# schreibfaul1/ESP32-Opus-Player

Measured on AMD Instinct MI355X. Metric: decoded 48 kHz stereo frames/sec/GPU (x real-time); HBM GB/s vs roofline, higher is better.
Workload: dtype int32 fixed-point (int16/int32 with 64-bit products); 1 GPU; celt_fb_stereo_64k; streams_per_gpu=65536

## Files before the change

### esp32-opus-player_amd/csrc/og_celt_packed.hpp

```cpp
#pragma once
#include <stddef.h>
#include "og_celt_bands.hpp"

namespace og {

#if defined(OG_RECON_TIGHT) && !defined(OG_HOST_EMUL)
constexpr bool PM_PACKED = true;
#else
constexpr bool PM_PACKED = false;
#endif

#ifdef OG_HOST_EMUL
OG_DEV u32 pk_perm(u32 hi, u32 lo, u32 sel) {
    const u64 v = (u64)hi << 32 | lo;
    u32 r = 0;
    for (int b = 0; b < 4; b++) r |= (u32)((v >> (8 * ((sel >> (8 * b)) & 7u))) & 0xffu) << (8 * b);
    return r;
}
OG_DEV i32 pk_dot2(u32 a, u32 b, i32 acc) {
    return (i32)((u32)acc + (u32)((i32)(i16)a * (i32)(i16)b) + (u32)(((i32)a >> 16) * ((i32)b >> 16)));
}
OG_DEV i32 pk_dot2_fits(u32 a, u32 b, i32 acc) { return pk_dot2(a, b, acc); }
OG_DEV u32 pk_add16(u32 a, u32 b) { return ((a + b) & 0xffffu) | ((a & 0xffff0000u) + (b & 0xffff0000u)); }
OG_DEV u32 pk_sub16(u32 a, u32 b) { return ((a - b) & 0xffffu) | ((a & 0xffff0000u) - (b & 0xffff0000u)); }
#else
typedef unsigned short og_u16x2 __attribute__((ext_vector_type(2)));
OG_DEV u32 pk_perm(u32 hi, u32 lo, u32 sel) { return __builtin_amdgcn_perm(hi, lo, sel); }
OG_DEV i32 pk_dot2(u32 a, u32 b, i32 acc) { return rs_dot2(a, b, acc); }
OG_DEV i32 pk_dot2_fits(u32 a, u32 b, i32 acc) {
    return __builtin_amdgcn_sdot2(__builtin_bit_cast(og_i16x2, a), __builtin_bit_cast(og_i16x2, b), acc, true);
}
OG_DEV u32 pk_add16(u32 a, u32 b) { return __builtin_bit_cast(u32, __builtin_bit_cast(og_u16x2, a) + __builtin_bit_cast(og_u16x2, b)); }
OG_DEV u32 pk_sub16(u32 a, u32 b) { return __builtin_bit_cast(u32, __builtin_bit_cast(og_u16x2, a) - __builtin_bit_cast(og_u16x2, b)); }
#endif
OG_DEV u32 pk_lolo(u32 a, u32 b) { return pk_perm(b, a, 0x05040100u); }
OG_DEV u32 pk_hihi(u32 a, u32 b) { return pk_perm(b, a, 0x07060302u); }
OG_DEV u32 pk_pair(i32 lo, i32 hi) { return ((u32)lo & 0xffffu) | (u32)hi << 16; }
OG_DEV u32 pk_q15(i32 lo, i32 hi) { return (((u32)lo >> 15) & 0xffffu) | (((u32)hi << 1) & 0xffff0000u); }
OG_DEV u32 pk_shr(i32 lo, i32 hi, int s) { return pk_pair(lo >> s, hi >> s); }

struct W4 { u32 w[4]; };
#ifdef OG_HOST_EMUL
template <typename T>
OG_DEV T pk_ld(const i16 *p) {
    T v;
    memcpy(&v, p, sizeof(T));
    return v;
}
OG_DEV W4 ldw4(const i16 *p) { return pk_ld<W4>(p); }
OG_DEV void stw4(i16 *p, const W4 &r) { memcpy(p, &r, sizeof(r)); }
#else
typedef i32 og_v4i __attribute__((ext_vector_type(4)));
template <typename T>
OG_DEV T pk_ld(const i16 *p) { return *reinterpret_cast<const T *>(p); }
OG_DEV W4 ldw4(const i16 *p) {
    const og_v4i v = *reinterpret_cast<const og_v4i *>(p);
    return W4{{(u32)v.x, (u32)v.y, (u32)v.z, (u32)v.w}};
}
OG_DEV void stw4(i16 *p, const W4 &r) { *reinterpret_cast<og_v4i *>(p) = og_v4i{(i32)r.w[0], (i32)r.w[1], (i32)r.w[2], (i32)r.w[3]}; }
#endif

#ifdef OG_HOST_EMUL
struct W2 { u32 w[2]; };
#else
struct alignas(8) W2 { u32 w[2]; };
#endif

constexpr u32 HAAR_SUM = 23170u | 23170u << 16, HAAR_DIF = 23170u | (u32)(u16)(-23170) << 16;
OG_DEV void pk_haar_words(u32 &x, u32 &y) {
    const u32 p = pk_lolo(x, y), q = pk_hihi(x, y);
    x = pk_q15(pk_dot2_fits(p, HAAR_SUM, 16384), pk_dot2_fits(q, HAAR_SUM, 16384));
    y = pk_q15(pk_dot2_fits(p, HAAR_DIF, 16384), pk_dot2_fits(q, HAAR_DIF, 16384));
}
OG_DEV void pk_haar8_1(W4 &r) {
    i32 s[4], d[4];
#pragma unroll
    for (int m = 0; m < 4; m++) {
        s[m] = pk_dot2_fits(r.w[m], HAAR_SUM, 16384);
        d[m] = pk_dot2_fits(r.w[m], HAAR_DIF, 16384);
    }
#pragma unroll
    for (int m = 0; m < 4; m++) r.w[m] = pk_q15(s[m], d[m]);
}
OG_DEV void pk_haar8_2(W4 &r) { pk_haar_words(r.w[0], r.w[1]); pk_haar_words(r.w[2], r.w[3]); }
OG_DEV void pk_haar8_4(W4 &r) { pk_haar_words(r.w[0], r.w[2]); pk_haar_words(r.w[1], r.w[3]); }
OG_DEV void pk_haar16(W4 &a, W4 &b) {
#pragma unroll
    for (int m = 0; m < 4; m++) pk_haar_words(a.w[m], b.w[m]);
}

static_assert(V_X % 8 == 0 && 960 % 8 == 0, "a channel's spectrum starts 16-byte aligned, its bands at multiples of 8 coefficients");
OG_DEV W4 pk_gather(const i16 *x, int N, int gj, int ls, bool had) {
    W4 r;
    if (ls == 2) {
        const int n0 = N >> 2;
        const i16 *p = x + 2 * gj;
        const u32 r0 = pk_ld<u32>(p + (had ? 3 : 0) * n0), r1 = pk_ld<u32>(p + (had ? 0 : 1) * n0);
        const u32 r2 = pk_ld<u32>(p + 2 * n0), r3 = pk_ld<u32>(p + (had ? 1 : 3) * n0);
        r.w[0] = pk_lolo(r0, r1);
        r.w[1] = pk_lolo(r2, r3);
        r.w[2] = pk_hihi(r0, r1);
        r.w[3] = pk_hihi(r2, r3);
    } else if (ls == 3) {
        const int n0 = N >> 3;
        const i16 *p = x + gj;
        const u32 rows = had ? 0x25163407u : 0x76543210u;
#pragma unroll
        for (int m = 0; m < 4; m++)
            r.w[m] = (u32)pk_ld<u16>(p + (int)((rows >> (8 * m)) & 15u) * n0) | (u32)pk_ld<u16>(p + (int)((rows >> (8 * m + 4)) & 15u) * n0) << 16;
    } else if (ls == 1) {
        const int n0 = N >> 1;
        const i16 *p = x + 4 * gj;
        const W2 a = pk_ld<W2>(p + (had ? n0 : 0)), b = pk_ld<W2>(p + (had ? 0 : n0));
        r.w[0] = pk_lolo(a.w[0], b.w[0]);
        r.w[1] = pk_hihi(a.w[0], b.w[0]);
        r.w[2] = pk_lolo(a.w[1], b.w[1]);
        r.w[3] = pk_hihi(a.w[1], b.w[1]);
    } else {
        const int stride = 1 << ls, n0 = N >> ls;
        i32 v[8];
#pragma unroll
        for (int k = 0; k < 8; k++) {
            const int inter = 8 * gj + k, j = inter >> ls, i = inter & (stride - 1);
            v[k] = x[(had ? ordery(stride, i) : i) * n0 + j];
        }
#pragma unroll
        for (int m = 0; m < 4; m++) r.w[m] = pk_pair(v[2 * m], v[2 * m + 1]);
    }
    return r;
}

OG_DEV void pk_merge_sums(const W4 &a, const W4 &b, i32 &xp, i32 &side) {
#pragma unroll
    for (int m = 0; m < 4; m++) {
        xp = pk_dot2(b.w[m], a.w[m], xp);
        side = pk_dot2(b.w[m], b.w[m], side);
    }
}
OG_DEV void pk_merge_apply(W4 &a, W4 &b, i32 mid, i32 lgain, i32 rgain, int kl, int kr, bool inv) {
    const u32 m_lo = (u32)mid & 0xffffu, m_hi = (u32)mid << 16;
    const u32 l_lo = (u32)lgain & 0xffffu, l_hi = (u32)lgain << 16, r_lo = (u32)rgain & 0xffffu, r_hi = (u32)rgain << 16;
    const i32 rl = (1 << (kl + 1)) >> 1, rr = (1 << (kr + 1)) >> 1;
#pragma unroll
    for (int m = 0; m < 4; m++) {
        const u32 l = pk_q15(pk_dot2_fits(a.w[m], m_lo, 16384), pk_dot2_fits(a.w[m], m_hi, 16384));
        const u32 d = pk_sub16(l, b.w[m]), s = pk_add16(l, b.w[m]);
        a.w[m] = pk_shr(pk_dot2_fits(d, l_lo, rl), pk_dot2_fits(d, l_hi, rl), kl + 1);
        const u32 y = pk_shr(pk_dot2_fits(s, r_lo, rr), pk_dot2_fits(s, r_hi, rr), kr + 1);
        b.w[m] = inv ? pk_sub16(0u, y) : y;
    }
}
OG_DEV W4 pk_neg(const W4 &a) { return W4{{pk_sub16(0u, a.w[0]), pk_sub16(0u, a.w[1]), pk_sub16(0u, a.w[2]), pk_sub16(0u, a.w[3])}}; }

static_assert(RING % 8 == 0 && 120 % 8 == 0 && OVERLAP / 2 % 4 == 0, "ring pieces of 4 samples: whole, and never across the wrap");
static_assert(offsetof(CeltState, ring) % 16 == 0 && offsetof(CeltState, tail) % 16 == 0 && sizeof(CeltState) % 16 == 0 &&
              sizeof(((CeltState *)nullptr)->tail[0]) % 16 == 0, "the ring and the tails are 16-byte aligned");
static_assert(V_SYN % 8 == 0, "the synthesis buffer is 16-byte aligned in the working set");
struct P4 { i32 v[4]; };
OG_DEV P4 pk_ld4(const i32 *p) {
#ifdef OG_HOST_EMUL
    P4 r;
    memcpy(&r, p, sizeof(r));
    return r;
#else
    const og_v4i v = *reinterpret_cast<const og_v4i *>(p);
    return P4{{v.x, v.y, v.z, v.w}};
#endif
}
OG_DEV void pk_st4(i32 *p, const P4 &r) {
#ifdef OG_HOST_EMUL
    memcpy(p, &r, sizeof(r));
#else
    *reinterpret_cast<og_v4i *>(p) = og_v4i{r.v[0], r.v[1], r.v[2], r.v[3]};
#endif
}
OG_DEV void pk_ring_tail_store(i32 *ring, i32 *tail, const i32 *sy, int pos, int n) {
    OG_FOR_LANES(p, n / 4) pk_st4(&ring[(pos + 4 * p) & RING_MASK], pk_ld4(&sy[4 * p]));
    OG_FOR_LANES(p, OVERLAP / 2 / 4) pk_st4(&tail[4 * p], pk_ld4(&sy[n + 4 * p]));
}

}
```

### esp32-opus-player_amd/csrc/og_celt_recon_pm.hpp

```cpp
#pragma once

namespace og {

struct PmLds {
    u32 jdesc[2 * NBANDS];
    u32 jaux[2 * NBANDS];
    u32 bw0[NBANDS], bw1[NBANDS], bw2[NBANDS];
    i32 scale[NBANDS];
    u32 mpar[NBANDS][2];
    u16 jcm[2 * NBANDS];
    u8 binband[100], binoff[100];
};
#ifdef OG_RECON_TIGHT
constexpr int V_PART = V_IY;
static_assert(sizeof(PmLds) <= sizeof(i16) * (V_IY - V_NORM) && 800 <= sizeof(i16) * (V_WIN - V_IY), "the phase-major tables");
#else
constexpr int V_PART = V_NORM + 600;
static_assert(sizeof(PmLds) <= sizeof(i16) * 600 && 600 + 400 <= 1248, "the phase-major tables overlay the folding-history rows");
#endif
OG_DEV PmLds &PM() { return *reinterpret_cast<PmLds *>(&S.v[V_NORM]); }
typedef i32 PmPart[2];
OG_DEV PmPart *pm_part() { return reinterpret_cast<PmPart *>(&S.v[V_PART]); }

enum {
    JD_VALID = 1, JD_FILL = 2,
    JD_PERM_SHIFT = 2 , JD_HAD = 1 << 5,
    JD_STEP_SHIFT = 8
};

struct V8 { i32 v[8]; };
OG_DEV V8 ld8(int pos) {
    V8 r;
#ifdef OG_HOST_EMUL
    for (int k = 0; k < 8; k++) r.v[k] = S.v[pos + k];
#else
    const og_v4i p = *reinterpret_cast<const og_v4i *>(&S.v[pos]);
    r.v[0] = (i32)(i16)p.x; r.v[1] = p.x >> 16; r.v[2] = (i32)(i16)p.y; r.v[3] = p.y >> 16;
    r.v[4] = (i32)(i16)p.z; r.v[5] = p.z >> 16; r.v[6] = (i32)(i16)p.w; r.v[7] = p.w >> 16;
#endif
    return r;
}
OG_DEV void st8(int pos, const V8 &r) {
#ifdef OG_HOST_EMUL
    for (int k = 0; k < 8; k++) S.v[pos + k] = (i16)r.v[k];
#else
    og_v4i p;
    p.x = (i32)(((u32)r.v[0] & 0xffffu) | (u32)r.v[1] << 16); p.y = (i32)(((u32)r.v[2] & 0xffffu) | (u32)r.v[3] << 16);
    p.z = (i32)(((u32)r.v[4] & 0xffffu) | (u32)r.v[5] << 16); p.w = (i32)(((u32)r.v[6] & 0xffffu) | (u32)r.v[7] << 16);
    *reinterpret_cast<og_v4i *>(&S.v[pos]) = p;
#endif
}
OG_DEV void haar_pair(i32 &a, i32 &b) {
    const i32 t1 = mul16(23170, a), t2 = mul16(23170, b);
    a = tr16(pshr32(t1 + t2, 15));
    b = tr16(pshr32(t1 - t2, 15));
}
template <int S_>
OG_DEV void haar8(V8 &r) {
#pragma unroll
    for (int i = 0; i < 8; i++)
        if (!(i & S_)) haar_pair(r.v[i], r.v[i + S_]);
}

template <bool PACKED> struct PmHold { typedef V8 type; };
template <> struct PmHold<true> { typedef W4 type; };

struct PmGrp { int band, job, x, gj, N; u32 jd; };
constexpr int PM_GROUPS = 100;
OG_DEV PmGrp pm_group(int g) {
    const PmLds &P = PM();
    PmGrp r;
    const int ch = g >= PM_GROUPS, bin = g - PM_GROUPS * ch;
    r.band = P.binband[bin];
    r.gj = P.binoff[bin];
    r.job = 2 * r.band + ch;
    r.jd = P.jdesc[r.job];
    r.x = V_X + 960 * ch + 8 * (bin - r.gj);
    r.N = (int)(P.bw1[r.band] >> 22) & 255;
    return r;
}

OG_DEV u32 pm_setup_jobs(const ParseRec *rec, int C, int B, u32 &fill_lo, u32 &fill_hi, int &dual_end, int start = 0, bool bw_staged = false) {
    PmLds &P = PM();
    OG_LSYNC();
    OG_FOR_LANES(bin, PM_GROUPS) {
        P.binband[bin] = rom_bin2band[bin];
        P.binoff[bin] = rom_binoff[bin];
    }
    OG_FOR_LANES(i, 2 * NBANDS) {
        P.jdesc[i] = 0;
        P.jcm[i] = 0;
    }
    OG_LSYNC();
    u32 tfm = 0, flo = 0, fhi = 0, de = 0;
    const int logBf = ilog2(B);
    OG_FOR_LANES(l, 2 * NBANDS) {
        const int band = l >> 1, jb = l & 1, coded = band >= start;
#ifdef OG_RECON_TIGHT
        const int bw = !coded ? 0 : bw_staged ? (int)S.band_w_row()[band] : (int)rec->band_w[band];
#else
        const int bw = coded ? (int)rec->band_w[band] : 0;
#endif
        const u32 *wp = rec->words + bw;
        const u32 w0 = coded ? wp[0] : 0u, w1 = coded ? wp[1] : 0u, w2 = coded ? wp[2] : 0u, w3 = coded ? wp[3] : 0u, jw0 = coded ? wp[4] : 0u;
        const int N = (int)(w1 >> 22) & 255;
        const int stereo = (w0 & BW_STEREO) != 0, dual = (w0 & BW_DUAL) != 0, mid_first = (w0 & BW_MID_FIRST) != 0;
        const int njobs = !coded ? 0 : (stereo || dual) ? 2 : 1;
        if (jb == 0) {
            P.bw0[band] = w0;
            P.bw1[band] = w1;
            P.bw2[band] = w2;
            P.scale[band] = (i32)(i16)(w3 & 0xffff);
            if (w0 & BW_DUAL_END) de |= 1u << band;
        }
        const int exists = jb < njobs;
        const int ch = dual ? jb : stereo ? (((jb == 0) == mid_first) ? 0 : 1) : 0;
        const int jpos = bw + 4 + (jb ? 1 + 2 * (int)(jw0 & 31) : 0);
        u32 jw = jw0;
        if (jb && exists) jw = rec->words[OG_MIN(jpos, REC_WORDS_CAP - 1)];
        const int n_fill = (int)(jw & 31), n_pvq = (int)(jw >> JW_NPVQ_SHIFT) & 31;
        P.jaux[l] = (u32)jpos | (u32)ch << 16 | (u32)exists << 17 | (u32)(exists && n_fill > 0) << 18 | (u32)(n_pvq > 0) << 19;
        if (exists) {
            int tf_change = (int)((w0 >> BW_TF_SHIFT) & 7) - 4;
            int recombine = tf_change > 0 ? tf_change : 0, time_divide = 0;
            int logB = logBf - recombine, N_B = (N >> logBf) << recombine;
            while ((N_B & 1) == 0 && tf_change < 0) {
                logB++;
                N_B >>= 1;
                time_divide++;
                tf_change++;
            }
            const int logB0 = logB;
            u32 jd = JD_VALID;
            if (logB0 > 0) jd |= (u32)(logB0 + recombine) << JD_PERM_SHIFT | (B == 1 ? JD_HAD : 0);
            int step = 0;
            for (int k = 0; k < time_divide; k++, step++) jd |= (u32)(logB0 - 1 - k + 1) << (JD_STEP_SHIFT + 4 * step);
            for (int k = 0; k < recombine; k++, step++) jd |= (u32)(k + 1) << (JD_STEP_SHIFT + 4 * step);
            if (n_fill > 0) {
                jd |= JD_FILL;
                if (l < 32) flo |= 1u << l; else fhi |= 1u << (l - 32);
            } else {
                if (logB0 > 0) tfm |= 1u;
                for (int k = 0; k < 3; k++) {
                    const int c = (int)(jd >> (JD_STEP_SHIFT + 4 * k)) & 15;
                    if (c) tfm |= 1u << (1 + 4 * k + (c - 1));
                }
                u32 cm = n_pvq ? S.job_mask_row()[l] : 0u;
                for (int k = 0; k < time_divide; k++) {
                    logB--;
                    cm |= cm >> (1 << logB);
                }
                for (int k = 0; k < recombine; k++) {
                    const u32 c4 = cm & 0xF;
                    cm = ((c4 & 1) * 0x03) | ((c4 >> 1 & 1) * 0x0C) | ((c4 >> 2 & 1) * 0x30) | ((c4 >> 3 & 1) * 0xC0);
                }
                logB += recombine;
                P.jcm[2 * band + ch] = (u16)(cm & ((1u << (1 << logB)) - 1));
            }
            P.jdesc[2 * band + ch] = jd;
        }
    }
    tfm = wave_or(tfm);
    fill_lo = wave_or(flo);
    fill_hi = wave_or(fhi);
    de = wave_or(de);
    dual_end = de ? ilog2((i32)de) : NBANDS + 1;
    OG_LSYNC();
    return tfm;
}

template <bool PACKED = PM_PACKED>
OG_DEV void pm_tf_undo(u32 tfm) {
    constexpr int NG = (2 * PM_GROUPS + OG_NLANES - 1) / OG_NLANES;
    typedef typename PmHold<PACKED>::type Hold;
    if (tfm & 1u) {
        Hold hold[NG];
        u8 mark[NG];
#pragma unroll
        for (int it = 0; it < NG; it++) {
            const int g = OG_LANE + it * OG_NLANES;
            mark[it] = 0;
            if (g < 2 * PM_GROUPS) {
                const PmGrp q = pm_group(g);
                const int ls = (int)(q.jd >> JD_PERM_SHIFT) & 7;
                if ((q.jd & JD_VALID) && !(q.jd & JD_FILL) && ls) {
                    const int stride = 1 << ls, n0 = q.N >> ls, had = (q.jd & JD_HAD) != 0;
                    if constexpr (PACKED)
                        hold[it] = pk_gather(&S.v[q.x], q.N, q.gj, ls, had);
                    else {
#pragma unroll
                        for (int k = 0; k < 8; k++) {
                            const int inter = 8 * q.gj + k, j = inter >> ls, i = inter & (stride - 1);
                            hold[it].v[k] = S.v[q.x + (had ? ordery(stride, i) : i) * n0 + j];
                        }
                    }
                    mark[it] = 1;
                }
            }
        }
        OG_LSYNC();
#pragma unroll
        for (int it = 0; it < NG; it++) {
            const int g = OG_LANE + it * OG_NLANES;
            if (mark[it]) {
                const PmGrp q = pm_group(g);
                if constexpr (PACKED) stw4(&S.v[q.x + 8 * q.gj], hold[it]);
                else st8(q.x + 8 * q.gj, hold[it]);
            }
        }
        OG_LSYNC();
    }
    if (tfm & (1u << (1 + 3))) {
#pragma unroll
        for (int it = 0; it < NG; it++) {
            const int g = OG_LANE + it * OG_NLANES;
            if (g < 2 * PM_GROUPS) {
                const PmGrp q = pm_group(g);
                if ((q.jd & JD_VALID) && !(q.jd & JD_FILL) && ((q.jd >> JD_STEP_SHIFT) & 15) == 4 && !(q.gj & 1)) {
                    if constexpr (PACKED) {
                        W4 a = ldw4(&S.v[q.x + 8 * q.gj]), b = ldw4(&S.v[q.x + 8 * q.gj + 8]);
                        pk_haar16(a, b);
                        stw4(&S.v[q.x + 8 * q.gj], a);
                        stw4(&S.v[q.x + 8 * q.gj + 8], b);
                    } else {
                        V8 a = ld8(q.x + 8 * q.gj), b = ld8(q.x + 8 * q.gj + 8);
#pragma unroll
                        for (int k = 0; k < 8; k++) haar_pair(a.v[k], b.v[k]);
                        st8(q.x + 8 * q.gj, a);
                        st8(q.x + 8 * q.gj + 8, b);
                    }
                }
            }
        }
        OG_LSYNC();
    }
    if (tfm & 0x0eeeu) {
#pragma unroll
        for (int it = 0; it < NG; it++) {
            const int g = OG_LANE + it * OG_NLANES;
            if (g < 2 * PM_GROUPS) {
                const PmGrp q = pm_group(g);
                const u32 steps = (q.jd & JD_VALID) && !(q.jd & JD_FILL) ? (q.jd >> JD_STEP_SHIFT) & 0xfffu : 0u;
                if (steps & 0x777u) {
                    if constexpr (PACKED) {
                        W4 r = ldw4(&S.v[q.x + 8 * q.gj]);
                        for (int k = 0; k < 3; k++) {
                            const int c = (int)(steps >> (4 * k)) & 15;
                            if (c == 1) pk_haar8_1(r);
                            else if (c == 2) pk_haar8_2(r);
                            else if (c == 3) pk_haar8_4(r);
                        }
                        stw4(&S.v[q.x + 8 * q.gj], r);
                    } else {
                        V8 r = ld8(q.x + 8 * q.gj);
                        for (int k = 0; k < 3; k++) {
                            const int c = (int)(steps >> (4 * k)) & 15;
                            if (c == 1) haar8<1>(r);
                            else if (c == 2) haar8<2>(r);
                            else if (c == 3) haar8<4>(r);
                        }
                        st8(q.x + 8 * q.gj, r);
                    }
                }
            }
        }
        OG_LSYNC();
    }
}

OG_DEV void pm_make_lowband(int dst, int p0, int n, int i, int use_y, int dual_end, int norm_offset = 0, int dup_n1 = 0, int dup_back = 0) {
    const PmLds &P = PM();
    OG_LSYNC();
    OG_FOR_LANES(j, n) {
        int r = p0 + j;
        const bool copied = dup_back && r >= dup_n1;
        if (copied) r -= dup_back;
        const int p = norm_offset + r, sb = P.binband[p >> 3];
        const i32 sc = P.scale[sb];
        i32 v;
        if (i >= dual_end && sb < dual_end && !copied)
            v = ((i32)(i16)mul16_q15(sc, S.v[V_X + p]) + (i32)(i16)mul16_q15(sc, S.v[V_X + 960 + p])) >> 1;
        else
            v = mul16_q15(sc, S.v[V_X + (use_y ? 960 : 0) + p]);
        S.v[dst + j] = (i16)v;
    }
    OG_LSYNC();
}

OG_DEV u32 pm_band_cm(int b, int c) {
    const PmLds &P = PM();
    const u32 w0 = (u32)OG_UNI(P.bw0[b]);
    if (w0 & BW_STEREO) return (u32)OG_UNI(P.jcm[2 * b]) | (u32)OG_UNI(P.jcm[2 * b + 1]);
    return (u32)OG_UNI(P.jcm[2 * b + ((w0 & BW_DUAL) ? c : 0)]);
}

OG_DEV void pm_fill_jobs(const u32 *words, const LcgTab &lcg, u32 fill_lo, u32 fill_hi, int C, int B, int dual_end, u32 &seed,
                         int start = 0) {
    const int norm_offset = 8 * rom_eband[start];
    const int dup_n1 = 8 * (rom_eband[start + 1] - rom_eband[start]), dup_n2 = 8 * (rom_eband[start + 2] - rom_eband[start + 1]);
    PmLds &P = PM();
    RecCur cur;
    cur.words = words;
    cur.w = 0;
    cur.base = -64;
    cur.leaf = 0;
    for (int l = 0; l < 2 * NBANDS; l++) {
        if (!((l < 32 ? fill_lo >> l : fill_hi >> (l - 32)) & 1u)) continue;
        OG_MARK(5);
        OG_STAT(20, 1);
        const int i = l >> 1, jb = l & 1;
        const u32 aux = (u32)OG_UNI(P.jaux[l]), w0 = (u32)OG_UNI(P.bw0[i]), w1 = (u32)OG_UNI(P.bw1[i]);
        const int ch = (int)(aux >> 16) & 1;
        const int eb0 = (int)(w1 >> 11) & 2047, N = (int)(w1 >> 22) & 255;
        const int tf_change = (int)((w0 >> BW_TF_SHIFT) & 7) - 4;
        const int stereo = (w0 & BW_STEREO) != 0, dual = (w0 & BW_DUAL) != 0;
        u32 x_cm, y_cm;
        if (w0 & BW_HAS_LOW) {
            const int fold_end = (int)(w0 >> BW_FOLD1_SHIFT) & 31;
            int fold_i = (int)(w0 >> BW_FOLD0_SHIFT) & 31;
            x_cm = y_cm = 0;
            do {
                x_cm |= pm_band_cm(fold_i, 0);
                y_cm |= pm_band_cm(fold_i, C - 1);
            } while (++fold_i < fold_end);
        } else
            x_cm = y_cm = (1u << B) - 1;
        i32 jfill;
        int want_low;
        if (dual) {
            jfill = (i32)(jb ? y_cm : x_cm);
            want_low = 1;
        } else {
            i32 fill0 = (i32)(x_cm | y_cm);
            if (stereo) {
                if (w0 & BW_THETA0) fill0 &= (1 << B) - 1;
                if (w0 & BW_THETA1) fill0 &= ((1 << B) - 1) << B;
            }
            jfill = ch ? fill0 >> B : fill0;
            want_low = !ch;
        }
        if (jfill == 0 && !(OG_UNI(P.jaux[l]) >> 19 & 1)) {
            OG_STAT(24, 1);
            continue;
        }
        cur.w = (int)(aux & 0xffff);
        OG_STAT(27, 1);
        const u32 jw = rec_word(cur);
        int low = -1;
        if ((w0 & BW_HAS_LOW) && want_low && (jw & JW_NEED_LOW)) {
            const int dup = (i == start + 1 && dup_n2 > dup_n1) ? dup_n2 - dup_n1 : 0;
            pm_make_lowband(V_IY, (int)(w1 & 2047), N, i, dual && ch, dual_end, norm_offset, dup_n1, dup);
            low = V_IY;
        }
        const u32 cm = recon_band_mono(cur, jw, lcg, tf_change, seed, V_X + 960 * ch + eb0, N, B, low, -1, 0, -1, jfill, l);
        if (OG_LANE == 0) P.jcm[2 * i + ch] = (u16)cm;
        OG_LSYNC();
    }
}

template <bool PACKED = PM_PACKED>
OG_DEV void pm_stereo_merge(int C) {
    PmLds &P = PM();
    if (C != 2) return;
    OG_LSYNC();
    const int eb_lo = rom_eband[OG_MIN(OG_LANE, NBANDS - 1)], eb_hi = rom_eband[OG_MIN(OG_LANE, NBANDS - 1) + 1];
    OG_FOR_LANES(g, PM_GROUPS) {
        const int band = P.binband[g];
        if (P.bw0[band] & BW_STEREO) {
            OG_STAT(29, 1);
            i32 xp = 0, side = 0;
            if constexpr (PACKED)
                pk_merge_sums(ldw4(&S.v[V_X + 8 * g]), ldw4(&S.v[V_X + 960 + 8 * g]), xp, side);
            else {
                const V8 a = ld8(V_X + 8 * g), b = ld8(V_X + 960 + 8 * g);
#pragma unroll
                for (int k = 0; k < 8; k++) {
                    xp += mul16(b.v[k], a.v[k]);
                    side += mul16(b.v[k], b.v[k]);
                }
            }
            pm_part()[g][0] = xp;
            pm_part()[g][1] = side;
        }
    }
    OG_LSYNC();
    OG_FOR_LANES(band, NBANDS) {
        const u32 w0 = P.bw0[band];
        if (w0 & BW_STEREO) {
            const int g0 = OG_NLANES > 1 ? eb_lo : rom_eband[band], g1 = OG_NLANES > 1 ? eb_hi : rom_eband[band + 1];
            i32 xp = 0, side = 0;
            for (int g = g0; g < g1; g++) {
                xp += pm_part()[g][0];
                side += pm_part()[g][1];
            }
            const i32 mid = (i32)(i16)(P.bw2[band] & 0xffff);
            xp = mul16x32_q15(mid, xp);
            const i32 mid2 = tr16(mid >> 1);
            const i32 El = mul16(mid2, mid2) + side - 2 * xp, Er = mul16(mid2, mid2) + side + 2 * xp;
            i32 mode = 1, lgain = 0, rgain = 0;
            int kl = 0, kr = 0;
            if (Er < 161061 || El < 161061)
                mode = 2;
            else {
                kl = ilog2(El) >> 1;
                kr = ilog2(Er) >> 1;
                lgain = rsqrt_norm(vshr32(El, (kl - 7) << 1));
                rgain = rsqrt_norm(vshr32(Er, (kr - 7) << 1));
                if (kl < 7) kl = 7;
                if (kr < 7) kr = 7;
            }
            if (w0 & BW_INV) mode |= 4;
            P.mpar[band][0] = (u32)(mode | kl << 8 | kr << 16);
            P.mpar[band][1] = ((u32)lgain & 0xffffu) | (u32)rgain << 16;
        } else
            P.mpar[band][0] = 0u;
    }
    OG_LSYNC();
    OG_FOR_LANES(g, PM_GROUPS) {
        const int band = P.binband[g];
        const i32 m0 = (i32)P.mpar[band][0];
        if (m0 & 3) {
            const u32 m1 = P.mpar[band][1];
            const i32 lgain = (i32)(i16)(m1 & 0xffff), rgain = (i32)m1 >> 16, mid = (i32)(i16)(P.bw2[band] & 0xffff);
            const int kl = (m0 >> 8) & 255, kr = (m0 >> 16) & 255;
            OG_STAT(37, 1);
            OG_STAT(38, (m0 & 2) != 0);
            if constexpr (PACKED) {
                W4 a = ldw4(&S.v[V_X + 8 * g]), b;
                if (m0 & 2)
                    b = (m0 & 4) ? pk_neg(a) : a;
                else {
                    b = ldw4(&S.v[V_X + 960 + 8 * g]);
                    pk_merge_apply(a, b, mid, lgain, rgain, kl, kr, (m0 & 4) != 0);
                    stw4(&S.v[V_X + 8 * g], a);
                }
                stw4(&S.v[V_X + 960 + 8 * g], b);
            } else {
                V8 a = ld8(V_X + 8 * g), b = ld8(V_X + 960 + 8 * g);
#pragma unroll
                for (int k = 0; k < 8; k++) {
                    i32 xo, yo;
                    if (m0 & 2) {
                        xo = a.v[k];
                        yo = a.v[k];
                    } else {
                        const i32 l = tr16(mul16_p15(mid, a.v[k])), r = b.v[k];
                        xo = tr16(pshr32(mul16(lgain, sub16(l, r)), kl + 1));
                        yo = tr16(pshr32(mul16(rgain, add16(l, r)), kr + 1));
                    }
                    a.v[k] = xo;
                    b.v[k] = (m0 & 4) ? tr16(-yo) : yo;
                }
                if (!(m0 & 2)) st8(V_X + 8 * g, a);
                st8(V_X + 960 + 8 * g, b);
            }
        }
    }
    OG_LSYNC();
}

OG_DEV void recon_all_bands_pm(const ParseRec *rec, LcgTab &lcg, int C, int shortBlocks, u32 &seed_io, int start = 0, bool bw_staged = false) {
    const int B = shortBlocks ? 8 : 1;
    u32 fill_lo, fill_hi, seed = seed_io;
    int dual_end;
    OG_MARK(3);
    const u32 tfm = pm_setup_jobs(rec, C, B, fill_lo, fill_hi, dual_end, start, bw_staged);
    if (fill_lo | fill_hi) lcg.hold();
#if defined(OG_HOST_EMUL) && defined(OG_STATS)
    {
        int n_fill_jobs = 0, w_prev = -1;
        bool close_pair = false;
        for (int l = 0; l < 2 * NBANDS; l++)
            if ((l < 32 ? fill_lo >> l : fill_hi >> (l - 32)) & 1u) {
                const int w = (int)(PM().jaux[l] & 0xffff);
                close_pair |= w_prev >= 0 && w - w_prev < 64;
                w_prev = w;
                n_fill_jobs++;
            }
        OG_STAT(33, n_fill_jobs == 0);
        OG_STAT(34, n_fill_jobs == 1);
        OG_STAT(35, n_fill_jobs >= 4);
        OG_STAT(36, close_pair);
    }
    {
        OG_STAT(25, (tfm & (1u << 4)) != 0);
        OG_STAT(28, (tfm & 0x0eeeu) != 0);
        for (int l = 0; l < 2 * NBANDS; l++) {
            const u32 jd = PM().jdesc[l];
            const int groups = (int)((PM().bw1[l >> 1] >> 22) & 255) / 8;
            if (!(jd & JD_VALID) || !(jd & ~(u32)(JD_VALID | JD_FILL))) continue;
            if (jd & JD_FILL) {
                OG_STAT(60, groups);
                continue;
            }
            const u32 steps = (jd >> JD_STEP_SHIFT) & 0xfffu;
            const int ls = (int)(jd >> JD_PERM_SHIFT) & 7, had = (jd & JD_HAD) != 0;
            OG_STAT(ls == 2 && had && steps == 0x012u ? 39
                    : ls == 3 && had && steps == 0x123u ? 43
                    : ls == 0 && steps == 0x321u ? 47
                    : ls == 3 && !had && steps == 0x001u ? 48
                    : ls == 3 && !had && steps == 0u ? 49
                    : ls == 4 && !had && steps == 0x004u ? 54
                    : 55, groups);
        }
    }
#endif
    OG_STAT(0, 1);
    OG_STAT(19, shortBlocks != 0);
    OG_STAT(21, tfm != 0);
    OG_STAT(22, (tfm & 1u) != 0);
    OG_STAT(23, (fill_lo | fill_hi) != 0);
    OG_MARK(8);
    if (tfm) pm_tf_undo(tfm);
    if (fill_lo | fill_hi) pm_fill_jobs(rec->words, lcg, fill_lo, fill_hi, C, B, dual_end, seed, start);
    OG_MARK(10);
    pm_stereo_merge(C);
    OG_MARK(4);
    OG_FOR_LANES(t, NBANDS * C) {
        const PmLds &P = PM();
        const int b = t / C, c = t - b * C;
        const u32 w0 = P.bw0[b];
        const u32 cm = (w0 & BW_STEREO) ? (u32)P.jcm[2 * b] | (u32)P.jcm[2 * b + 1] : (u32)P.jcm[2 * b + ((w0 & BW_DUAL) ? c : 0)];
        S.cmask_row()[t] = (u8)cm;
    }
    OG_LSYNC();
    seed_io = seed;
}

#ifdef OG_RECON_TIGHT
static_assert(sizeof(i32) * 2 * PM_GROUPS <= offsetof(PmLds, binband), "the groups' sums end before the bin tables");
static_assert(48 + 2 * 2 * NBANDS <= 200 && (V_TMP + 48) % 2 == 0, "r and the entries' words fit the scratch row");
OG_DEV void anti_collapse_pm(const LcgTab &lcg, int LM, int C, int size, int start, int end, u32 seed) {
    const PmLds &P = PM();
    const i16 *const rrow = anti_collapse_r(LM, C, start, end);
    u32 *const ent = reinterpret_cast<u32 *>(&S.v[V_TMP + 48]);
    i32 *const part = reinterpret_cast<i32 *>(&S.v[V_NORM]);
    const int NE = C * NBANDS;
    OG_STAT(32, 1);
    u32 run = 0;
    (void)run;
    OG_FOR_LANES(e, OG_NLANES > 1 ? OG_NLANES : NE) {
        const int i = C == 2 ? e >> 1 : e;
        int draws = 0;
        if (e < NE && i >= start && i < end) {
            const int cnt = __builtin_popcount(~(u32)S.cmask_row()[e] & 0xffu);
            draws = cnt * (rom_eband[i + 1] - rom_eband[i]);
            OG_STAT(30, cnt);
            OG_STAT(31, cnt != 0);
        }
#ifdef OG_HOST_EMUL
        const u32 before = run;
        run += (u32)draws;
#else
        const u32 before = (u32)(wave_scan_add(draws) - draws);
#endif
        if (e < NE) ent[e] = lcg_skip(seed, before);
    }
    OG_LSYNC();
    OG_FOR_LANES(t, C * PM_GROUPS) {
        const int c = t >= PM_GROUPS, g = t - PM_GROUPS * c;
        const int i = P.binband[g], j = P.binoff[g], e = i * C + c;
        const u32 clr = (i >= start && i < end) ? ~(u32)S.cmask_row()[e] & 0xffu : 0u;
        if (clr) {
            const int N0 = rom_eband[i + 1] - rom_eband[i];
            const i32 r = rrow[c * NBANDS + i];
            const u32 base = ent[e];
            V8 x = ld8(V_X + c * size + 8 * g);
            int at = j;
            i32 ss = 0;
#pragma unroll
            for (int k = 0; k < 8; k++) {
                const u32 s = lcg.at(base, at);
                if ((clr >> k) & 1u) {
                    x.v[k] = (i16)((s & 0x8000) ? r : -r);
                    at += N0;
                }
                ss += mul16(x.v[k], x.v[k]);
            }
            st8(V_X + c * size + 8 * g, x);
            part[t] = ss;
        }
    }
    OG_LSYNC();
    OG_FOR_LANES(e, NE) {
        const int i = C == 2 ? e >> 1 : e, c = e - i * C;
        u32 w = 0;
        if (i >= start && i < end && (~(u32)S.cmask_row()[e] & 0xffu)) {
            const int g0 = rom_eband[i], g1 = rom_eband[i + 1];
            i32 E = 1;
            for (int g = g0; g < g1; g++) E += part[c * PM_GROUPS + g];
            const int k = ilog2(E) >> 1;
            const i32 t = vshr32(E, 2 * (k - 7));
            const i32 gn = tr16(mul16_p15(rsqrt_norm(t), 32767));
            w = ((u32)gn & 0xffffu) | (u32)((k + 1) & 63) << 16 | 1u << 31;
        }
        ent[e] = w;
    }
    OG_LSYNC();
    OG_FOR_LANES(t, C * PM_GROUPS) {
        const int c = t >= PM_GROUPS, g = t - PM_GROUPS * c;
        const u32 w = ent[P.binband[g] * C + c];
        if (w) {
            const i32 gn = (i32)(i16)(w & 0xffff);
            const int sh = (int)(w >> 16) & 63;
            V8 x = ld8(V_X + c * size + 8 * g);
#pragma unroll
            for (int k = 0; k < 8; k++) x.v[k] = (i16)pshr32(mul16(gn, x.v[k]), sh);
            st8(V_X + c * size + 8 * g, x);
        }
    }
    OG_LSYNC();
}
#endif

}
```

Before: 52.50 million frames/s.

## Route fill-job band TF transforms through packed group-wise haar/permute path

In packed mode, fill jobs no longer call recon_band_mono. They plan the TF recombine/time-divide themselves, apply the forward haar and permute to the lowband in 8-coefficient groups using packed dot2 ops, and decode the leaves. They then undo the TF transform per job with group-wise gather, haar and scatter, and rebuild the collapse mask from the plan. This replaces the generic scalar per-coefficient TF loops with vectorized packed LDS accesses, at the cost of extra barriers and a new scatter path. The change also refactors pm_tf_undo onto shared helpers and adds a host-only census instrument.

```diff
diff --git a/esp32-opus-player_amd/csrc/og_celt_packed.hpp b/esp32-opus-player_amd/csrc/og_celt_packed.hpp
--- a/esp32-opus-player_amd/csrc/og_celt_packed.hpp
+++ b/esp32-opus-player_amd/csrc/og_celt_packed.hpp
@@ -130,6 +130,45 @@
     return r;
 }
 
+#ifdef OG_HOST_EMUL
+template <typename T>
+OG_DEV void pk_st(i16 *p, const T &v) { memcpy(p, &v, sizeof(T)); }
+#else
+template <typename T>
+OG_DEV void pk_st(i16 *p, const T &v) { *reinterpret_cast<T *>(p) = v; }
+#endif
+OG_DEV void pk_scatter(i16 *x, int N, int gj, int ls, bool had, const W4 &r) {
+    if (ls == 2) {
+        const int n0 = N >> 2;
+        i16 *p = x + 2 * gj;
+        pk_st<u32>(p + (had ? 3 : 0) * n0, pk_lolo(r.w[0], r.w[2]));
+        pk_st<u32>(p + (had ? 0 : 1) * n0, pk_hihi(r.w[0], r.w[2]));
+        pk_st<u32>(p + 2 * n0, pk_lolo(r.w[1], r.w[3]));
+        pk_st<u32>(p + (had ? 1 : 3) * n0, pk_hihi(r.w[1], r.w[3]));
+    } else if (ls == 3) {
+        const int n0 = N >> 3;
+        i16 *p = x + gj;
+        const u32 rows = had ? 0x25163407u : 0x76543210u;
+#pragma unroll
+        for (int m = 0; m < 4; m++) {
+            pk_st<u16>(p + (int)((rows >> (8 * m)) & 15u) * n0, (u16)r.w[m]);
+            pk_st<u16>(p + (int)((rows >> (8 * m + 4)) & 15u) * n0, (u16)(r.w[m] >> 16));
+        }
+    } else if (ls == 1) {
+        const int n0 = N >> 1;
+        i16 *p = x + 4 * gj;
+        pk_st<W2>(p + (had ? n0 : 0), W2{{pk_lolo(r.w[0], r.w[1]), pk_lolo(r.w[2], r.w[3])}});
+        pk_st<W2>(p + (had ? 0 : n0), W2{{pk_hihi(r.w[0], r.w[1]), pk_hihi(r.w[2], r.w[3])}});
+    } else {
+        const int stride = 1 << ls, n0 = N >> ls;
+#pragma unroll
+        for (int k = 0; k < 8; k++) {
+            const int inter = 8 * gj + k, j = inter >> ls, i = inter & (stride - 1);
+            x[(had ? ordery(stride, i) : i) * n0 + j] = (i16)(u16)(r.w[k >> 1] >> (16 * (k & 1)));
+        }
+    }
+}
+
 OG_DEV void pk_merge_sums(const W4 &a, const W4 &b, i32 &xp, i32 &side) {
 #pragma unroll
     for (int m = 0; m < 4; m++) {
diff --git a/esp32-opus-player_amd/csrc/og_celt_recon_pm.hpp b/esp32-opus-player_amd/csrc/og_celt_recon_pm.hpp
--- a/esp32-opus-player_amd/csrc/og_celt_recon_pm.hpp
+++ b/esp32-opus-player_amd/csrc/og_celt_recon_pm.hpp
@@ -1,4 +1,8 @@
 #pragma once
+
+#if defined(OG_HOST_EMUL) && defined(OG_STATS) && defined(OG_FILL_CENSUS)
+extern long long og_fill_census[32];
+#endif
 
 namespace og {
 
@@ -62,8 +66,60 @@
         if (!(i & S_)) haar_pair(r.v[i], r.v[i + S_]);
 }
 
-template <bool PACKED> struct PmHold { typedef V8 type; };
-template <> struct PmHold<true> { typedef W4 type; };
+template <bool PACKED> struct PmHold {
+    typedef V8 type;
+    static OG_MEMBER V8 ld(int pos) { return ld8(pos); }
+    static OG_MEMBER V8 gather(int x, int N, int gj, int ls, bool had) {
+        const int stride = 1 << ls, n0 = N >> ls;
+        V8 r;
+#pragma unroll
+        for (int k = 0; k < 8; k++) {
+            const int inter = 8 * gj + k, j = inter >> ls, i = inter & (stride - 1);
+            r.v[k] = S.v[x + (had ? ordery(stride, i) : i) * n0 + j];
+        }
+        return r;
+    }
+};
+template <> struct PmHold<true> {
+    typedef W4 type;
+    static OG_MEMBER W4 ld(int pos) { return ldw4(&S.v[pos]); }
+    static OG_MEMBER W4 gather(int x, int N, int gj, int ls, bool had) { return pk_gather(&S.v[x], N, gj, ls, had); }
+};
+OG_DEV void pm_grp_st(int pos, const V8 &r) { st8(pos, r); }
+OG_DEV void pm_grp_st(int pos, const W4 &r) { stw4(&S.v[pos], r); }
+OG_DEV void pm_grp_scatter(int x, int N, int gj, int ls, bool had, const V8 &r) {
+    const int stride = 1 << ls, n0 = N >> ls;
+#pragma unroll
+    for (int k = 0; k < 8; k++) {
+        const int inter = 8 * gj + k, j = inter >> ls, i = inter & (stride - 1);
+        S.v[x + (had ? ordery(stride, i) : i) * n0 + j] = (i16)r.v[k];
+    }
+}
+OG_DEV void pm_grp_scatter(int x, int N, int gj, int ls, bool had, const W4 &r) { pk_scatter(&S.v[x], N, gj, ls, had, r); }
+OG_DEV V8 pm_grp_steps(V8 r, u32 steps) {
+    for (int k = 0; k < 3; k++) {
+        const int c = (int)(steps >> (4 * k)) & 15;
+        if (c == 1) haar8<1>(r);
+        else if (c == 2) haar8<2>(r);
+        else if (c == 3) haar8<4>(r);
+    }
+    return r;
+}
+OG_DEV W4 pm_grp_steps(W4 r, u32 steps) {
+    for (int k = 0; k < 3; k++) {
+        const int c = (int)(steps >> (4 * k)) & 15;
+        if (c == 1) pk_haar8_1(r);
+        else if (c == 2) pk_haar8_2(r);
+        else if (c == 3) pk_haar8_4(r);
+    }
+    return r;
+}
+OG_DEV u32 pm_steps_reversed(u32 steps) { return (steps & 0x0f0u) | (steps >> 8 & 15u) | (steps & 15u) << 8; }
+OG_DEV void pm_grp_pair(V8 &a, V8 &b) {
+#pragma unroll
+    for (int k = 0; k < 8; k++) haar_pair(a.v[k], b.v[k]);
+}
+OG_DEV void pm_grp_pair(W4 &a, W4 &b) { pk_haar16(a, b); }
 
 struct PmGrp { int band, job, x, gj, N; u32 jd; };
 constexpr int PM_GROUPS = 100;
@@ -172,7 +228,8 @@
 template <bool PACKED = PM_PACKED>
 OG_DEV void pm_tf_undo(u32 tfm) {
     constexpr int NG = (2 * PM_GROUPS + OG_NLANES - 1) / OG_NLANES;
-    typedef typename PmHold<PACKED>::type Hold;
+    typedef PmHold<PACKED> G;
+    typedef typename G::type Hold;
     if (tfm & 1u) {
         Hold hold[NG];
         u8 mark[NG];
@@ -184,16 +241,7 @@
                 const PmGrp q = pm_group(g);
                 const int ls = (int)(q.jd >> JD_PERM_SHIFT) & 7;
                 if ((q.jd & JD_VALID) && !(q.jd & JD_FILL) && ls) {
-                    const int stride = 1 << ls, n0 = q.N >> ls, had = (q.jd & JD_HAD) != 0;
-                    if constexpr (PACKED)
-                        hold[it] = pk_gather(&S.v[q.x], q.N, q.gj, ls, had);
-                    else {
-#pragma unroll
-                        for (int k = 0; k < 8; k++) {
-                            const int inter = 8 * q.gj + k, j = inter >> ls, i = inter & (stride - 1);
-                            hold[it].v[k] = S.v[q.x + (had ? ordery(stride, i) : i) * n0 + j];
-                        }
-                    }
+                    hold[it] = G::gather(q.x, q.N, q.gj, ls, (q.jd & JD_HAD) != 0);
                     mark[it] = 1;
                 }
             }
@@ -204,8 +252,7 @@
             const int g = OG_LANE + it * OG_NLANES;
             if (mark[it]) {
                 const PmGrp q = pm_group(g);
-                if constexpr (PACKED) stw4(&S.v[q.x + 8 * q.gj], hold[it]);
-                else st8(q.x + 8 * q.gj, hold[it]);
+                pm_grp_st(q.x + 8 * q.gj, hold[it]);
             }
         }
         OG_LSYNC();
@@ -217,18 +264,10 @@
             if (g < 2 * PM_GROUPS) {
                 const PmGrp q = pm_group(g);
                 if ((q.jd & JD_VALID) && !(q.jd & JD_FILL) && ((q.jd >> JD_STEP_SHIFT) & 15) == 4 && !(q.gj & 1)) {
-                    if constexpr (PACKED) {
-                        W4 a = ldw4(&S.v[q.x + 8 * q.gj]), b = ldw4(&S.v[q.x + 8 * q.gj + 8]);
-                        pk_haar16(a, b);
-                        stw4(&S.v[q.x + 8 * q.gj], a);
-                        stw4(&S.v[q.x + 8 * q.gj + 8], b);
-                    } else {
-                        V8 a = ld8(q.x + 8 * q.gj), b = ld8(q.x + 8 * q.gj + 8);
-#pragma unroll
-                        for (int k = 0; k < 8; k++) haar_pair(a.v[k], b.v[k]);
-                        st8(q.x + 8 * q.gj, a);
-                        st8(q.x + 8 * q.gj + 8, b);
-                    }
+                    Hold a = G::ld(q.x + 8 * q.gj), b = G::ld(q.x + 8 * q.gj + 8);
+                    pm_grp_pair(a, b);
+                    pm_grp_st(q.x + 8 * q.gj, a);
+                    pm_grp_st(q.x + 8 * q.gj + 8, b);
                 }
             }
         }
@@ -242,30 +281,104 @@
                 const PmGrp q = pm_group(g);
                 const u32 steps = (q.jd & JD_VALID) && !(q.jd & JD_FILL) ? (q.jd >> JD_STEP_SHIFT) & 0xfffu : 0u;
                 if (steps & 0x777u) {
-                    if constexpr (PACKED) {
-                        W4 r = ldw4(&S.v[q.x + 8 * q.gj]);
-                        for (int k = 0; k < 3; k++) {
-                            const int c = (int)(steps >> (4 * k)) & 15;
-                            if (c == 1) pk_haar8_1(r);
-                            else if (c == 2) pk_haar8_2(r);
-                            else if (c == 3) pk_haar8_4(r);
-                        }
-                        stw4(&S.v[q.x + 8 * q.gj], r);
-                    } else {
-                        V8 r = ld8(q.x + 8 * q.gj);
-                        for (int k = 0; k < 3; k++) {
-                            const int c = (int)(steps >> (4 * k)) & 15;
-                            if (c == 1) haar8<1>(r);
-                            else if (c == 2) haar8<2>(r);
-                            else if (c == 3) haar8<4>(r);
-                        }
-                        st8(q.x + 8 * q.gj, r);
-                    }
+                    Hold r = G::ld(q.x + 8 * q.gj);
+                    pm_grp_st(q.x + 8 * q.gj, pm_grp_steps(r, steps));
                 }
             }
         }
         OG_LSYNC();
     }
+}
+
+constexpr int PM_JOB_GROUPS = 22;
+constexpr int PM_JOB_TRIPS = (PM_JOB_GROUPS + OG_NLANES - 1) / OG_NLANES;
+template <bool PACKED = PM_PACKED>
+OG_DEV void pm_job_tf_undo(int x, int N, u32 jd) {
+    typedef PmHold<PACKED> G;
+    typedef typename G::type Hold;
+    const int ls = (int)(jd >> JD_PERM_SHIFT) & 7, groups = N >> 3;
+    const bool had = (jd & JD_HAD) != 0;
+    const u32 steps = (jd >> JD_STEP_SHIFT) & 0xfffu;
+    if (!ls && !steps) return;
+    const bool pairs = (steps & 15u) == 4u;
+    Hold hold[PM_JOB_TRIPS];
+    OG_LSYNC();
+#pragma unroll
+    for (int it = 0; it < PM_JOB_TRIPS; it++) {
+        const int gj = OG_LANE + it * OG_NLANES;
+        if (gj < groups) {
+            if (ls) hold[it] = G::gather(x, N, gj, ls, had);
+            else if (!pairs) hold[it] = G::ld(x + 8 * gj);
+        }
+    }
+    if (ls) OG_LSYNC();
+    if (pairs) {
+        if (ls) {
+#pragma unroll
+            for (int it = 0; it < PM_JOB_TRIPS; it++) {
+                const int gj = OG_LANE + it * OG_NLANES;
+                if (gj < groups) pm_grp_st(x + 8 * gj, hold[it]);
+            }
+            OG_LSYNC();
+        }
+        OG_FOR_LANES(gp, groups >> 1) {
+            Hold a = G::ld(x + 16 * gp), b = G::ld(x + 16 * gp + 8);
+            pm_grp_pair(a, b);
+            a = pm_grp_steps(a, steps);
+            b = pm_grp_steps(b, steps);
+            pm_grp_st(x + 16 * gp, a);
+            pm_grp_st(x + 16 * gp + 8, b);
+        }
+    } else {
+#pragma unroll
+        for (int it = 0; it < PM_JOB_TRIPS; it++) {
+            const int gj = OG_LANE + it * OG_NLANES;
+            if (gj < groups) {
+                pm_grp_st(x + 8 * gj, pm_grp_steps(hold[it], steps));
+            }
+        }
+    }
+    OG_LSYNC();
+}
+
+template <bool PACKED = PM_PACKED>
+OG_DEV void pm_job_tf_fwd(int low, int N, u32 jd, bool reverse) {
+    typedef PmHold<PACKED> G;
+    typedef typename G::type Hold;
+    const int ls = (int)(jd >> JD_PERM_SHIFT) & 7, groups = N >> 3;
+    const bool had = (jd & JD_HAD) != 0;
+    const u32 steps = (jd >> JD_STEP_SHIFT) & 0xfffu;
+    if (!ls && !steps) return;
+    const u32 fwd_steps = reverse ? pm_steps_reversed(steps) : steps;
+    Hold hold[PM_JOB_TRIPS];
+    OG_LSYNC();
+    if ((steps & 15u) == 4u) {
+        OG_FOR_LANES(gp, groups >> 1) {
+            Hold a = G::ld(low + 16 * gp), b = G::ld(low + 16 * gp + 8);
+            pm_grp_pair(a, b);
+            pm_grp_st(low + 16 * gp, a);
+            pm_grp_st(low + 16 * gp + 8, b);
+        }
+        OG_LSYNC();
+    }
+#pragma unroll
+    for (int it = 0; it < PM_JOB_TRIPS; it++) {
+        const int gj = OG_LANE + it * OG_NLANES;
+        if (gj < groups) {
+            hold[it] = G::ld(low + 8 * gj);
+            hold[it] = pm_grp_steps(hold[it], fwd_steps);
+            if (!ls) pm_grp_st(low + 8 * gj, hold[it]);
+        }
+    }
+    if (ls) {
+        OG_LSYNC();
+#pragma unroll
+        for (int it = 0; it < PM_JOB_TRIPS; it++) {
+            const int gj = OG_LANE + it * OG_NLANES;
+            if (gj < groups) pm_grp_scatter(low, N, gj, ls, had, hold[it]);
+        }
+    }
+    OG_LSYNC();
 }
 
 OG_DEV void pm_make_lowband(int dst, int p0, int n, int i, int use_y, int dual_end, int norm_offset = 0, int dup_n1 = 0, int dup_back = 0) {
@@ -292,6 +405,59 @@
     const u32 w0 = (u32)OG_UNI(P.bw0[b]);
     if (w0 & BW_STEREO) return (u32)OG_UNI(P.jcm[2 * b]) | (u32)OG_UNI(P.jcm[2 * b + 1]);
     return (u32)OG_UNI(P.jcm[2 * b + ((w0 & BW_DUAL) ? c : 0)]);
+}
+
+struct PmTfPlan { int recombine, time_divide, logB0; };
+OG_DEV PmTfPlan pm_tf_plan(int tf_change, int N, int B, i32 &fill) {
+    PmTfPlan p;
+    p.recombine = tf_change > 0 ? tf_change : 0;
+    p.time_divide = 0;
+    for (int k = 0; k < p.recombine; k++) {
+        const int lo = fill & 0xF, hi = fill >> 4;
+        const int tl = (lo & 3 ? 1 : 0) | (lo & 12 ? 2 : 0), th = (hi & 3 ? 1 : 0) | (hi & 12 ? 2 : 0);
+        fill = tl | th << 2;
+    }
+    int logB = ilog2(B), N_B = (N >> logB) << p.recombine;
+    logB -= p.recombine;
+    while ((N_B & 1) == 0 && tf_change < 0) {
+        fill |= fill << (1 << logB);
+        logB++;
+        N_B >>= 1;
+        p.time_divide++;
+        tf_change++;
+    }
+    p.logB0 = logB;
+    return p;
+}
+OG_DEV u32 pm_tf_cm_up(const PmTfPlan &p, u32 cm) {
+    int logB = p.logB0;
+    for (int k = 0; k < p.time_divide; k++) {
+        logB--;
+        cm |= cm >> (1 << logB);
+    }
+    for (int k = 0; k < p.recombine; k++) {
+        const u32 c4 = cm & 0xF;
+        cm = ((c4 & 1) * 0x03) | ((c4 >> 1 & 1) * 0x0C) | ((c4 >> 2 & 1) * 0x30) | ((c4 >> 3 & 1) * 0xC0);
+    }
+    logB += p.recombine;
+    return cm & ((1u << (1 << logB)) - 1);
+}
+template <bool PACKED = PM_PACKED>
+OG_DEV u32 pm_fill_job_band(RecCur &cur, u32 jw, const LcgTab &lcg, int tf_change, u32 jd, u32 &seed, int x, int N, int B, int low, i32 fill,
+                            int job) {
+    if constexpr (!PACKED)
+        return recon_band_mono(cur, jw, lcg, tf_change, seed, x, N, B, low, -1, 0, -1, fill, job);
+    else {
+        if (!(jw & JW_NEED_LOW)) low = -1;
+        const PmTfPlan plan = pm_tf_plan(tf_change, N, B, fill);
+        if (low >= 0) pm_job_tf_fwd<true>(low, N, jd, plan.time_divide > 0);
+        OG_MARK(6);
+        const u32 cm = recon_job_leaves(cur, lcg, jw, seed, x, low, fill, job);
+        OG_MARK(8);
+        pm_job_tf_undo<true>(x, N, jd);
+        OG_MARK(9);
+        return pm_tf_cm_up(plan, cm);
+    }
 }
 
 OG_DEV void pm_fill_jobs(const u32 *words, const LcgTab &lcg, u32 fill_lo, u32 fill_hi, int C, int B, int dual_end, u32 &seed,
@@ -352,7 +518,40 @@
             pm_make_lowband(V_IY, (int)(w1 & 2047), N, i, dual && ch, dual_end, norm_offset, dup_n1, dup);
             low = V_IY;
         }
-        const u32 cm = recon_band_mono(cur, jw, lcg, tf_change, seed, V_X + 960 * ch + eb0, N, B, low, -1, 0, -1, jfill, l);
+        const u32 jd = (u32)OG_UNI(P.jdesc[2 * i + ch]);
+#if defined(OG_HOST_EMUL) && defined(OG_STATS) && defined(OG_FILL_CENSUS)
+        {
+            const u32 steps = (jd >> JD_STEP_SHIFT) & 0xfffu;
+            const int ls = (int)(jd >> JD_PERM_SHIFT) & 7, had = (jd & JD_HAD) != 0;
+            const int cls = !ls && !steps ? 0
+                            : ls == 2 && had && steps == 0x012u ? 1
+                            : ls == 3 && had && steps == 0x123u ? 2
+                            : ls == 0 && steps == 0x321u ? 3
+                            : ls == 3 && !had && steps == 0x001u ? 4
+                            : ls == 3 && !had && steps == 0u ? 5
+                            : ls == 4 && !had && steps == 0x004u ? 6
+                            : 7;
+            const int nsteps = (steps & 15u ? 1 : 0) + (steps & 0xf0u ? 1 : 0) + (steps & 0xf00u ? 1 : 0);
+            const int haar_trips = nsteps * ((N / 2 + 63) / 64), had_trips = ls ? 2 * ((N + 63) / 64) : 0;
+            og_fill_census[0 + cls]++;
+            og_fill_census[16] += N / 8;
+            og_fill_census[17] += cls ? N / 8 : 0;
+            og_fill_census[18] += nsteps;
+            og_fill_census[19] += ls != 0;
+            og_fill_census[20] += haar_trips;
+            og_fill_census[21] += had_trips;
+            if (low >= 0) {
+                og_fill_census[8 + cls]++;
+                og_fill_census[22] += cls ? N / 8 : 0;
+                og_fill_census[23] += nsteps;
+                og_fill_census[24] += ls != 0;
+                og_fill_census[25] += haar_trips;
+                og_fill_census[26] += had_trips;
+                og_fill_census[27] += ((N + 63) / 64);
+            }
+        }
+#endif
+        const u32 cm = pm_fill_job_band(cur, jw, lcg, tf_change, jd, seed, V_X + 960 * ch + eb0, N, B, low, jfill, l);
         if (OG_LANE == 0) P.jcm[2 * i + ch] = (u16)cm;
         OG_LSYNC();
     }
```

Result: no change. 52.50 million frames/s (-0.0%).
